# XiSHEN0220/RANSAC-Flow

Hardware: AMD Instinct MI355X
Metric: aligned image-pairs/sec @480×640, 1/2/4/8 MI355X; max-abs flow Δ vs ref (higher is better)
Workload: dtype f32

## Files before the change

ransac-flow_amd/csrc/stem.hip:

```cpp
#include "common.h"
#include "group.h"

namespace {

constexpr int TH = 4, TW = 16;
constexpr int CR = 2 * TH + 2, CC = 2 * TW + 2;
constexpr int PRW = CR + 2, PCL = CC + 2;
constexpr int CST = CC + 1;
constexpr int CPS = CR * CST + 1;
constexpr int NPX = CR * CC;
constexpr int NSUB = (NPX + 31) / 32;
constexpr int KKS = 14;
constexpr int MCH = 32;

struct StemArgs {
    const float* in; const float* wT; const float* scale; const float* shift; float* out;
    int N, H, W, Cout, Mpad, Ho, Wo, tilesH, tilesW, chGroups;
};

__device__ __forceinline__ int reflect1i(int i, int n) { return i < 0 ? -i : (i >= n ? 2 * n - 2 - i : i); }

__device__ __forceinline__ float umaxf(float x, float y) {
    const unsigned a = __float_as_uint(x), b = __float_as_uint(y);
    return __uint_as_float(a > b ? a : b);
}

__global__ __launch_bounds__(256) void stem_conv_maxblur_kernel(StemArgs a) {
    __shared__ float P[3][PRW][PCL];
    __shared__ float C[MCH * CPS];

    const int t = threadIdx.x, lane = t & 63, wave = t >> 6;
    const int lrow = lane >> 5, lcol = lane & 31;
    int bid = blockIdx.x;
    const int cg = bid % a.chGroups; bid /= a.chGroups;
    const int tw = bid % a.tilesW; bid /= a.tilesW;
    const int th = bid % a.tilesH;
    const int n = bid / a.tilesH;
    const int oh0 = th * TH, ow0 = tw * TW;
    const int cy0 = 2 * oh0 - 1, cx0 = 2 * ow0 - 1;
    const int m0 = cg * MCH;
    const size_t HW = (size_t)a.H * a.W;

    const float* inn = a.in + (size_t)n * 3 * HW;
    constexpr int NP = (3 * PRW * PCL + 255) / 256;
    float pv_[NP];
    bool pok[NP];
#pragma unroll
    for (int u = 0; u < NP; ++u) {
        const int idx = t + 256 * u;
        const int c = idx / (PRW * PCL), rem = idx - c * (PRW * PCL);
        const int pr = rem / PCL, pc = rem - pr * PCL;
        const int gy = cy0 - 1 + pr, gx = cx0 - 1 + pc;
        pok[u] = idx < 3 * PRW * PCL && (unsigned)gy < (unsigned)a.H && (unsigned)gx < (unsigned)a.W;
        pv_[u] = inn[pok[u] ? (size_t)c * HW + (size_t)gy * a.W + gx : 0];
    }
    float af[KKS];
#pragma unroll
    for (int kk = 0; kk < KKS; ++kk) af[kk] = a.wT[(size_t)(2 * kk + lrow) * a.Mpad + m0 + lcol];
    int koff[KKS];
#pragma unroll
    for (int kk = 0; kk < KKS; ++kk) {
        const int k = 2 * kk + lrow;
        const int c = k / 9, t9 = k - c * 9, kh = t9 / 3, kw = t9 - kh * 3;
        koff[kk] = k < 27 ? c * (PRW * PCL) + kh * PCL + kw : 0;
    }
    float sc[16], sh[16];
#pragma unroll
    for (int r = 0; r < 16; ++r) {
        const int ch = m0 + 4 * lrow + (r & 3) + 8 * (r >> 2);
        sc[r] = a.scale ? a.scale[ch] : 1.0f;
        sh[r] = a.shift ? a.shift[ch] : 0.0f;
    }
#pragma unroll
    for (int u = 0; u < NP; ++u)
        if (t + 256 * u < 3 * PRW * PCL) (&P[0][0][0])[t + 256 * u] = pok[u] ? pv_[u] : 0.0f;
    __syncthreads();

    const float* pf = &P[0][0][0];
    for (int s = wave; s < NSUB; s += 4) {
        const int p = s * 32 + lcol;
        const bool pv = p < NPX;
        const int pc = pv ? p : 0;
        const int py = pc / CC, px = pc - py * CC;
        const int pbase = py * PCL + px;
        f32x16 acc;
#pragma unroll
        for (int r = 0; r < 16; ++r) acc[r] = 0.0f;
#pragma unroll
        for (int kk = 0; kk < KKS; ++kk) {
            float b = pf[pbase + koff[kk]];
            if (kk == KKS - 1) b = lrow ? 0.0f : b;
            acc = __builtin_amdgcn_mfma_f32_32x32x2f32(af[kk], b, acc, 0, 0, 0);
        }
        if (pv) {
#pragma unroll
            for (int r = 0; r < 16; ++r) {
                float v = fmaf(acc[r], sc[r], sh[r]);
                v = v > 0.0f ? v : 0.0f;
                C[(4 * lrow + (r & 3) + 8 * (r >> 2)) * CPS + py * CST + px] = v;
            }
        }
    }
    __syncthreads();

    const float w3[3] = {0.25f, 0.5f, 0.25f};
    const int Hm = a.H - 1, Wm = a.W - 1;
    for (int b = t; b < MCH * (TH / 2) * (TW / 2); b += 256) {
        const int bx = b % (TW / 2), by = (b / (TW / 2)) % (TH / 2), ch = b / ((TW / 2) * (TH / 2));
        const int oh = oh0 + 2 * by, ow = ow0 + 2 * bx;
        if (oh >= a.Ho || ow >= a.Wo) continue;
        float* dst = a.out + ((size_t)n * a.Cout + m0 + ch) * a.Ho * a.Wo;
        const float* Cc = C + ch * CPS;
        const bool interior = oh >= 1 && 2 * oh + 3 <= Hm - 1 && ow >= 1 && 2 * ow + 3 <= Wm - 1 && oh + 1 < a.Ho && ow + 1 < a.Wo;
        if (interior) {
            const int ly = 2 * oh - 1 - cy0, lx = 2 * ow - 1 - cx0;
            float v[6][6];
#pragma unroll
            for (int y = 0; y < 6; ++y)
#pragma unroll
                for (int x = 0; x < 6; ++x) v[y][x] = Cc[(ly + y) * CST + lx + x];
            float hmx[5][6], M[5][5];
#pragma unroll
            for (int y = 0; y < 5; ++y)
#pragma unroll
                for (int x = 0; x < 6; ++x) hmx[y][x] = umaxf(v[y][x], v[y + 1][x]);
#pragma unroll
            for (int y = 0; y < 5; ++y)
#pragma unroll
                for (int x = 0; x < 5; ++x) M[y][x] = umaxf(hmx[y][x], hmx[y][x + 1]);
#pragma unroll
            for (int dy = 0; dy < 2; ++dy)
#pragma unroll
                for (int dx = 0; dx < 2; ++dx) {
                    float acc = 0.0f;
#pragma unroll
                    for (int i = 0; i < 3; ++i)
#pragma unroll
                        for (int j = 0; j < 3; ++j) acc = fmaf(M[2 * dy + i][2 * dx + j], w3[i] * w3[j], acc);
                    dst[(size_t)(oh + dy) * a.Wo + ow + dx] = acc;
                }
            continue;
        }
        for (int dy = 0; dy < 2; ++dy)
            for (int dx = 0; dx < 2; ++dx) {
                const int o_h = oh + dy, o_w = ow + dx;
                if (o_h >= a.Ho || o_w >= a.Wo) continue;
                float acc = 0.0f;
#pragma unroll
                for (int i = 0; i < 3; ++i) {
                    const int my = reflect1i(2 * o_h - 1 + i, Hm) - cy0;
#pragma unroll
                    for (int j = 0; j < 3; ++j) {
                        const int mx = reflect1i(2 * o_w - 1 + j, Wm) - cx0;
                        const float m = umaxf(umaxf(Cc[my * CST + mx], Cc[(my + 1) * CST + mx]), umaxf(Cc[my * CST + mx + 1], Cc[(my + 1) * CST + mx + 1]));
                        acc = fmaf(m, w3[i] * w3[j], acc);
                    }
                }
                dst[(size_t)o_h * a.Wo + o_w] = acc;
            }
    }
}


namespace r50 {
constexpr int TH = 5, TW = 16;
constexpr int CR = 2 * TH + 1, CC = 2 * TW + 1;
constexpr int PR = 2 * CR + 5, PCW = 2 * CC + 5;
constexpr int PHALF = 36, PST = 2 * PHALF + 2;
constexpr int CHALF = 17, CST = 40;
constexpr int NSUB = CR + 1;
constexpr int KKS = 74;
constexpr int MCH = 32;
__host__ __device__ constexpr int koff(int k) {
    return k >= 147 ? 0 : (k / 49) * (PR * PST) + ((k % 49) / 7) * PST + (((k % 49) % 7) & 1) * PHALF + (((k % 49) % 7) >> 1);
}
}

struct Stem7Args {
    const float* in; const float* wT; const float* scale; const float* shift; float* out;
    int N, H, W, Cout, Mpad, Hc, Wc, Hp, Wp, tilesH, tilesW, chGroups;
#ifdef RFX_TRACE
    long long* trace;
#endif
};
#ifdef RFX_TRACE
extern "C" long long* rfx_debug_trace_ptr();
#define RFX_STAMP7(i) do { if (threadIdx.x == 0 && a.trace) a.trace[(size_t)bx * 8 + (i)] = (long long)__builtin_amdgcn_s_memtime(); } while (0)
#else
#define RFX_STAMP7(i)
#endif

__device__ __forceinline__ void stem7_conv_maxpool_body(const Stem7Args& a, const unsigned bx) {
    constexpr int TH = r50::TH, TW = r50::TW, CR = r50::CR, CC = r50::CC, PR = r50::PR, PCW = r50::PCW, PHALF = r50::PHALF,
                  PST = r50::PST, CST = r50::CST, CHALF = r50::CHALF, NSUB = r50::NSUB, KKS = r50::KKS, MCH = r50::MCH;
    using r50::koff;
    __shared__ float P[3][PR][PST];
    __shared__ float C[MCH][CR][CST];

    const int t = threadIdx.x, lane = t & 63, wave = t >> 6;
    const int lrow = lane >> 5, lcol = lane & 31;
    int bid = (int)bx;
    const int cg_first = bid % a.chGroups;
    bid /= a.chGroups;
    const int tw = bid % a.tilesW; bid /= a.tilesW;
    const int th = bid % a.tilesH;
    const int n = bid / a.tilesH;
    const int oh0 = th * TH, ow0 = tw * TW;
    const int cy0 = 2 * oh0 - 1, cx0 = 2 * ow0 - 1;
    const int iy0 = 2 * cy0 - 3, ix0 = 2 * cx0 - 3;
    const size_t HW = (size_t)a.H * a.W;

    RFX_STAMP7(0);
    const float* inn = a.in + (size_t)n * 3 * HW;
    constexpr int NP = (3 * PR * PCW + 255) / 256;
    float pv_[NP];
    unsigned pok = 0;
    const int c_0 = t / (PR * PCW), rem_0 = t - c_0 * (PR * PCW), pr_0 = rem_0 / PCW, pc_0 = rem_0 - pr_0 * PCW;
    {
        int c = c_0, pr = pr_0, pc = pc_0;
#pragma unroll
        for (int u = 0; u < NP; ++u) {
            const int gy = iy0 + pr, gx = ix0 + pc;
            const bool ok = c < 3 && (unsigned)gy < (unsigned)a.H && (unsigned)gx < (unsigned)a.W;
            pok |= ok ? (1u << u) : 0u;
            pv_[u] = inn[ok ? (size_t)c * HW + (size_t)gy * a.W + gx : 0];
            pc += 256 % PCW; pr += 256 / PCW;
            if (pc >= PCW) { pc -= PCW; ++pr; }
            if (pr >= PR) { pr -= PR; ++c; }
        }
    }
    float af[KKS];
    __shared__ float s_bn[2][128];
    for (int c = t; c < a.Cout && c < 128; c += 256) {
        s_bn[0][c] = a.scale ? a.scale[c] : 1.0f;
        s_bn[1][c] = a.shift ? a.shift[c] : 0.0f;
    }
    auto load_weights = [&](int m0) {
        const float* wl = a.wT;
        asm volatile("" : "+s"(wl) :: "memory");
#pragma unroll
        for (int kk = 0; kk < KKS; ++kk) af[kk] = wl[(size_t)(2 * kk + lrow) * a.Mpad + m0 + lcol];
    };
    load_weights(cg_first * MCH);
    {
        int c = c_0, pr = pr_0, pc = pc_0;
#pragma unroll
        for (int u = 0; u < NP; ++u) {
            if (c < 3) P[c][pr][(pc & 1) * PHALF + (pc >> 1)] = ((pok >> u) & 1u) ? pv_[u] : 0.0f;
            pc += 256 % PCW; pr += 256 / PCW;
            if (pc >= PCW) { pc -= PCW; ++pr; }
            if (pr >= PR) { pr -= PR; ++c; }
        }
    }
    RFX_STAMP7(1);
    __syncthreads();
    RFX_STAMP7(2);

    auto channel_group = [&](const int cg) {
    const int m0 = cg * MCH;
    const float* pf = &P[0][0][0];
    for (int s = wave; s < NSUB; s += 4) {
        const bool pv = s < CR || lcol < CR;
        const int py = s < CR ? s : (lcol < CR ? lcol : 0), px = s < CR ? lcol : CC - 1;
        const int pbase = 2 * py * PST + px;
        f32x16 acc;
#pragma unroll
        for (int r = 0; r < 16; ++r) acc[r] = 0.0f;
#pragma unroll
        for (int kk = 0; kk < KKS; ++kk) {
            const int off = lrow ? koff(2 * kk + 1) : koff(2 * kk);
            float b = pf[pbase + off];
            if (kk == KKS - 1) b = lrow ? 0.0f : b;
            acc = __builtin_amdgcn_mfma_f32_32x32x2f32(af[kk], b, acc, 0, 0, 0);
        }
        if (pv) {
#pragma unroll
            for (int r = 0; r < 16; ++r) {
                const int chl = m0 + 4 * lrow + (r & 3) + 8 * (r >> 2);
                float v = fmaf(acc[r], s_bn[0][chl], s_bn[1][chl]);
                v = v > 0.0f ? v : 0.0f;
                C[4 * lrow + (r & 3) + 8 * (r >> 2)][py][(px & 1) * CHALF + (px >> 1)] = v;
            }
        }
    }
    RFX_STAMP7(3);
    __syncthreads();
    RFX_STAMP7(4);

    for (int o = t; o < MCH * TH * TW; o += 256) {
        const int owl = o % TW, ohl = (o / TW) % TH, ch = o / (TW * TH);
        const int oh = oh0 + ohl, ow = ow0 + owl;
        if (oh >= a.Hp || ow >= a.Wp) continue;
        float m = 0.0f;
#pragma unroll
        for (int i = 0; i < 3; ++i) {
            const int gy = cy0 + 2 * ohl + i;
#pragma unroll
            for (int j = 0; j < 3; ++j) {
                const int gx = cx0 + 2 * owl + j;
                const bool ok = (unsigned)gy < (unsigned)a.Hc && (unsigned)gx < (unsigned)a.Wc;
                const float v = C[ch][2 * ohl + i][(j & 1) * CHALF + owl + (j >> 1)];
                m = ok ? umaxf(m, v) : m;
            }
        }
        a.out[(((size_t)n * a.Cout + m0 + ch) * a.Hp + oh) * a.Wp + ow] = m;
    }
    RFX_STAMP7(5);
    };
#pragma unroll 1
    for (int cg = cg_first; cg < cg_first + 1; ++cg) channel_group(cg);
}

__global__ __launch_bounds__(256, 2) void stem7_conv_maxpool_kernel(Stem7Args a) {
    stem7_conv_maxpool_body(a, blockIdx.x);
}

__global__ __launch_bounds__(256, 2) void stem7_conv_maxpool_group_kernel(RfxGroupArgs<Stem7Args> g) {
    const unsigned y = blockIdx.y;
    if (blockIdx.x >= g.gx[y]) return;
    stem7_conv_maxpool_body(g.p[y], blockIdx.x);
}

static int stem7_group_launch(const void* blob, const unsigned* gx, int n, hipStream_t st) {
    return rfx_group_launch_impl<Stem7Args>(stem7_conv_maxpool_group_kernel, 256, blob, gx, n, st);
}

}

extern "C" int rfx_stem_conv3x3_maxblur_f32(const float* in, const float* wT, const float* scale, const float* shift,
                                            float* out, int N, int H, int W, int Cout, void* stream) {
    if (!in || !wT || !out || N <= 0 || H < 3 || W < 3 || Cout <= 0) return RFX_E_ARG;
    if (Cout % MCH != 0) return RFX_E_ARG;
    StemArgs a;
    a.in = in; a.wT = wT; a.scale = scale; a.shift = shift; a.out = out;
    a.N = N; a.H = H; a.W = W; a.Cout = Cout; a.Mpad = (Cout + 127) / 128 * 128;
    a.Ho = (H - 2) / 2 + 1; a.Wo = (W - 2) / 2 + 1;
    a.tilesH = (a.Ho + TH - 1) / TH; a.tilesW = (a.Wo + TW - 1) / TW; a.chGroups = Cout / MCH;
    const long long nwg = (long long)N * a.tilesH * a.tilesW * a.chGroups;
    if (nwg > 0x7fffffffLL) return RFX_E_LIMIT;
    hipLaunchKernelGGL(stem_conv_maxblur_kernel, dim3((unsigned)nwg), dim3(256), 0, rfx_stream(stream), a);
    RFX_LAUNCH_CHECK();
    return RFX_OK;
}

extern "C" int rfx_stem_conv7x7_maxpool_f32(const float* in, const float* wT, const float* scale, const float* shift,
                                            float* out, int N, int H, int W, int Cout, void* stream) {
    if (!in || !wT || !out || N <= 0 || H < 1 || W < 1 || Cout <= 0) return RFX_E_ARG;
    if (Cout % r50::MCH != 0) return RFX_E_ARG;
    if (Cout > 128) return RFX_E_LIMIT;
    Stem7Args a;
    a.in = in; a.wT = wT; a.scale = scale; a.shift = shift; a.out = out;
    a.N = N; a.H = H; a.W = W; a.Cout = Cout; a.Mpad = (Cout + 127) / 128 * 128;
    a.Hc = (H + 6 - 7) / 2 + 1; a.Wc = (W + 6 - 7) / 2 + 1;
    a.Hp = (a.Hc + 2 - 3) / 2 + 1; a.Wp = (a.Wc + 2 - 3) / 2 + 1;
    a.tilesH = (a.Hp + r50::TH - 1) / r50::TH; a.tilesW = (a.Wp + r50::TW - 1) / r50::TW; a.chGroups = Cout / r50::MCH;
    const long long nwg = (long long)N * a.tilesH * a.tilesW * a.chGroups;
    if (nwg > 0x7fffffffLL) return RFX_E_LIMIT;
#ifdef RFX_TRACE
    a.trace = rfx_debug_trace_ptr();
#endif
    if (rfx_group_recording()) return rfx_group_record(&stem7_group_launch, &a, sizeof(a), (unsigned)nwg);
    hipLaunchKernelGGL(stem7_conv_maxpool_kernel, dim3((unsigned)nwg), dim3(256), 0, rfx_stream(stream), a);
    RFX_LAUNCH_CHECK();
    return RFX_OK;
}
```

Baseline: 164.4.

## Loop channel groups inside stem blocks and fuse horizontal maxpool via DPP

Both stem kernels now stage each input tile into LDS once and loop over all channel groups inside one workgroup, instead of launching a separate workgroup per channel group that reloads the same patch. The next group's weights are prefetched during the pooling phase. The 7x7 stem also does the horizontal 3-wide max inside the MFMA epilogue using DPP row shifts, and keeps a small side buffer for tile-edge columns, which shrinks the LDS intermediate and the pooling pass. The cost is fewer workgroups (a factor of chGroups) and therefore less parallelism, plus an extra barrier per group.

```diff
diff --git a/ransac-flow_amd/csrc/stem.hip b/ransac-flow_amd/csrc/stem.hip
--- a/ransac-flow_amd/csrc/stem.hip
+++ b/ransac-flow_amd/csrc/stem.hip
@@ -32,13 +32,11 @@
     const int t = threadIdx.x, lane = t & 63, wave = t >> 6;
     const int lrow = lane >> 5, lcol = lane & 31;
     int bid = blockIdx.x;
-    const int cg = bid % a.chGroups; bid /= a.chGroups;
     const int tw = bid % a.tilesW; bid /= a.tilesW;
     const int th = bid % a.tilesH;
     const int n = bid / a.tilesH;
     const int oh0 = th * TH, ow0 = tw * TW;
     const int cy0 = 2 * oh0 - 1, cx0 = 2 * ow0 - 1;
-    const int m0 = cg * MCH;
     const size_t HW = (size_t)a.H * a.W;
 
     const float* inn = a.in + (size_t)n * 3 * HW;
@@ -55,8 +53,11 @@
         pv_[u] = inn[pok[u] ? (size_t)c * HW + (size_t)gy * a.W + gx : 0];
     }
     float af[KKS];
-#pragma unroll
-    for (int kk = 0; kk < KKS; ++kk) af[kk] = a.wT[(size_t)(2 * kk + lrow) * a.Mpad + m0 + lcol];
+    auto load_weights = [&](const int m0) {
+#pragma unroll
+        for (int kk = 0; kk < KKS; ++kk) af[kk] = a.wT[(size_t)(2 * kk + lrow) * a.Mpad + m0 + lcol];
+    };
+    load_weights(0);
     int koff[KKS];
 #pragma unroll
     for (int kk = 0; kk < KKS; ++kk) {
@@ -64,6 +65,17 @@
         const int c = k / 9, t9 = k - c * 9, kh = t9 / 3, kw = t9 - kh * 3;
         koff[kk] = k < 27 ? c * (PRW * PCL) + kh * PCL + kw : 0;
     }
+#pragma unroll
+    for (int u = 0; u < NP; ++u)
+        if (t + 256 * u < 3 * PRW * PCL) (&P[0][0][0])[t + 256 * u] = pok[u] ? pv_[u] : 0.0f;
+    __syncthreads();
+
+    const float* pf = &P[0][0][0];
+    const float w3[3] = {0.25f, 0.5f, 0.25f};
+    const int Hm = a.H - 1, Wm = a.W - 1;
+#pragma unroll 1
+    for (int cg = 0; cg < a.chGroups; ++cg) {
+    const int m0 = cg * MCH;
     float sc[16], sh[16];
 #pragma unroll
     for (int r = 0; r < 16; ++r) {
@@ -71,18 +83,13 @@
         sc[r] = a.scale ? a.scale[ch] : 1.0f;
         sh[r] = a.shift ? a.shift[ch] : 0.0f;
     }
-#pragma unroll
-    for (int u = 0; u < NP; ++u)
-        if (t + 256 * u < 3 * PRW * PCL) (&P[0][0][0])[t + 256 * u] = pok[u] ? pv_[u] : 0.0f;
-    __syncthreads();
-
-    const float* pf = &P[0][0][0];
     for (int s = wave; s < NSUB; s += 4) {
         const int p = s * 32 + lcol;
         const bool pv = p < NPX;
         const int pc = pv ? p : 0;
         const int py = pc / CC, px = pc - py * CC;
-        const int pbase = py * PCL + px;
+        int pbase = py * PCL + px;
+        asm volatile("" : "+v"(pbase));
         f32x16 acc;
 #pragma unroll
         for (int r = 0; r < 16; ++r) acc[r] = 0.0f;
@@ -102,9 +109,8 @@
         }
     }
     __syncthreads();
-
-    const float w3[3] = {0.25f, 0.5f, 0.25f};
-    const int Hm = a.H - 1, Wm = a.W - 1;
+    if (cg + 1 < a.chGroups) load_weights(m0 + MCH);
+
     for (int b = t; b < MCH * (TH / 2) * (TW / 2); b += 256) {
         const int bx = b % (TW / 2), by = (b / (TW / 2)) % (TH / 2), ch = b / ((TW / 2) * (TH / 2));
         const int oh = oh0 + 2 * by, ow = ow0 + 2 * bx;
@@ -159,6 +165,8 @@
                 dst[(size_t)o_h * a.Wo + o_w] = acc;
             }
     }
+    __syncthreads();
+    }
 }
 
 
@@ -167,7 +175,8 @@
 constexpr int CR = 2 * TH + 1, CC = 2 * TW + 1;
 constexpr int PR = 2 * CR + 5, PCW = 2 * CC + 5;
 constexpr int PHALF = 36, PST = 2 * PHALF + 2;
-constexpr int CHALF = 17, CST = 40;
+constexpr int HPS = CR * TW + 4;
+constexpr int SPS = 24;
 constexpr int NSUB = CR + 1;
 constexpr int KKS = 74;
 constexpr int MCH = 32;
@@ -185,23 +194,33 @@
 };
 #ifdef RFX_TRACE
 extern "C" long long* rfx_debug_trace_ptr();
-#define RFX_STAMP7(i) do { if (threadIdx.x == 0 && a.trace) a.trace[(size_t)bx * 8 + (i)] = (long long)__builtin_amdgcn_s_memtime(); } while (0)
+#define RFX_NOW7() ((long long)__builtin_amdgcn_s_memtime())
+#define RFX_STAMP7(i) do { if (threadIdx.x == 0 && a.trace) a.trace[(size_t)bx * 8 + (i)] = RFX_NOW7(); } while (0)
+#define RFX_PUT7(i, v) do { if (threadIdx.x == 0 && a.trace) a.trace[(size_t)bx * 8 + (i)] = (v); } while (0)
+#define RFX_TRACE7(x) x
 #else
 #define RFX_STAMP7(i)
+#define RFX_PUT7(i, v)
+#define RFX_TRACE7(x)
 #endif
 
+template <int N>
+__device__ __forceinline__ unsigned row_shl0(unsigned v) {
+    return (unsigned)__builtin_amdgcn_update_dpp(0, (int)v, 0x100 + N, 0xf, 0xf, true);
+}
+
 __device__ __forceinline__ void stem7_conv_maxpool_body(const Stem7Args& a, const unsigned bx) {
-    constexpr int TH = r50::TH, TW = r50::TW, CR = r50::CR, CC = r50::CC, PR = r50::PR, PCW = r50::PCW, PHALF = r50::PHALF,
-                  PST = r50::PST, CST = r50::CST, CHALF = r50::CHALF, NSUB = r50::NSUB, KKS = r50::KKS, MCH = r50::MCH;
+    constexpr int TH = r50::TH, TW = r50::TW, CR = r50::CR, PR = r50::PR, PCW = r50::PCW, PHALF = r50::PHALF,
+                  PST = r50::PST, HPS = r50::HPS, SPS = r50::SPS, NSUB = r50::NSUB, KKS = r50::KKS, MCH = r50::MCH;
     using r50::koff;
     __shared__ float P[3][PR][PST];
-    __shared__ float C[MCH][CR][CST];
+    __shared__ float Hx[MCH * HPS];
+    __shared__ float Sd[MCH * SPS];
+    __shared__ float s_bn[2][128];
 
     const int t = threadIdx.x, lane = t & 63, wave = t >> 6;
     const int lrow = lane >> 5, lcol = lane & 31;
     int bid = (int)bx;
-    const int cg_first = bid % a.chGroups;
-    bid /= a.chGroups;
     const int tw = bid % a.tilesW; bid /= a.tilesW;
     const int th = bid % a.tilesH;
     const int n = bid / a.tilesH;
@@ -229,19 +248,17 @@
             if (pr >= PR) { pr -= PR; ++c; }
         }
     }
-    float af[KKS];
-    __shared__ float s_bn[2][128];
     for (int c = t; c < a.Cout && c < 128; c += 256) {
         s_bn[0][c] = a.scale ? a.scale[c] : 1.0f;
         s_bn[1][c] = a.shift ? a.shift[c] : 0.0f;
     }
-    auto load_weights = [&](int m0) {
-        const float* wl = a.wT;
-        asm volatile("" : "+s"(wl) :: "memory");
-#pragma unroll
-        for (int kk = 0; kk < KKS; ++kk) af[kk] = wl[(size_t)(2 * kk + lrow) * a.Mpad + m0 + lcol];
+    float af[KKS];
+    auto load_weights = [&](const int m0) {
+        const unsigned voff = (unsigned)(lrow * a.Mpad + m0 + lcol);
+#pragma unroll
+        for (int kk = 0; kk < KKS; ++kk) af[kk] = (a.wT + (size_t)(2 * kk) * a.Mpad)[voff];
     };
-    load_weights(cg_first * MCH);
+    load_weights(0);
     {
         int c = c_0, pr = pr_0, pc = pc_0;
 #pragma unroll
@@ -255,14 +272,20 @@
     RFX_STAMP7(1);
     __syncthreads();
     RFX_STAMP7(2);
-
-    auto channel_group = [&](const int cg) {
+    RFX_TRACE7(long long tr_mark = RFX_NOW7(); long long tr_mfma = 0; long long tr_pool = 0;)
+
+    const float* pf = &P[0][0][0];
+#pragma unroll 1
+    for (int cg = 0; cg < a.chGroups; ++cg) {
     const int m0 = cg * MCH;
-    const float* pf = &P[0][0][0];
     for (int s = wave; s < NSUB; s += 4) {
-        const bool pv = s < CR || lcol < CR;
-        const int py = s < CR ? s : (lcol < CR ? lcol : 0), px = s < CR ? lcol : CC - 1;
-        const int pbase = 2 * py * PST + px;
+        const bool rowt = s < CR;
+        const int cl = lcol & 15;
+        const bool pv = rowt || cl < CR;
+        const int py = rowt ? s : (cl < CR ? cl : 0), px = rowt ? lcol : 16 + (lcol & 16);
+        int pbase = 2 * py * PST + px;
+        asm volatile("" : "+v"(pbase));
+        const bool ok = pv && (unsigned)(cy0 + py) < (unsigned)a.Hc && (unsigned)(cx0 + px) < (unsigned)a.Wc;
         f32x16 acc;
 #pragma unroll
         for (int r = 0; r < 16; ++r) acc[r] = 0.0f;
@@ -273,42 +296,56 @@
             if (kk == KKS - 1) b = lrow ? 0.0f : b;
             acc = __builtin_amdgcn_mfma_f32_32x32x2f32(af[kk], b, acc, 0, 0, 0);
         }
-        if (pv) {
+        if (rowt) {
+            unsigned hm[16];
 #pragma unroll
             for (int r = 0; r < 16; ++r) {
                 const int chl = m0 + 4 * lrow + (r & 3) + 8 * (r >> 2);
                 float v = fmaf(acc[r], s_bn[0][chl], s_bn[1][chl]);
                 v = v > 0.0f ? v : 0.0f;
-                C[4 * lrow + (r & 3) + 8 * (r >> 2)][py][(px & 1) * CHALF + (px >> 1)] = v;
+                const unsigned u = ok ? __float_as_uint(v) : 0u;
+                const unsigned u1 = row_shl0<1>(u), u2 = row_shl0<2>(u);
+                const unsigned m1 = u > u1 ? u : u1;
+                hm[r] = m1 > u2 ? m1 : u2;
             }
-        }
-    }
-    RFX_STAMP7(3);
-    __syncthreads();
-    RFX_STAMP7(4);
+            if (!(lcol & 1)) {
+#pragma unroll
+                for (int r = 0; r < 16; ++r)
+                    Hx[(4 * lrow + (r & 3) + 8 * (r >> 2)) * HPS + py * TW + (lcol >> 1)] = __uint_as_float(hm[r]);
+            }
+        } else if (pv) {
+#pragma unroll
+            for (int r = 0; r < 16; ++r) {
+                const int chl = m0 + 4 * lrow + (r & 3) + 8 * (r >> 2);
+                float v = fmaf(acc[r], s_bn[0][chl], s_bn[1][chl]);
+                v = v > 0.0f ? v : 0.0f;
+                Sd[(4 * lrow + (r & 3) + 8 * (r >> 2)) * SPS + (lcol >> 4) * 12 + py] = ok ? v : 0.0f;
+            }
+        }
+    }
+    __syncthreads();
+    RFX_TRACE7(const long long tr_a = RFX_NOW7(); tr_mfma += tr_a - tr_mark; tr_mark = tr_a;)
+    if (cg + 1 < a.chGroups) load_weights(m0 + MCH);
 
     for (int o = t; o < MCH * TH * TW; o += 256) {
         const int owl = o % TW, ohl = (o / TW) % TH, ch = o / (TW * TH);
         const int oh = oh0 + ohl, ow = ow0 + owl;
         if (oh >= a.Hp || ow >= a.Wp) continue;
-        float m = 0.0f;
-#pragma unroll
-        for (int i = 0; i < 3; ++i) {
-            const int gy = cy0 + 2 * ohl + i;
-#pragma unroll
-            for (int j = 0; j < 3; ++j) {
-                const int gx = cx0 + 2 * owl + j;
-                const bool ok = (unsigned)gy < (unsigned)a.Hc && (unsigned)gx < (unsigned)a.Wc;
-                const float v = C[ch][2 * ohl + i][(j & 1) * CHALF + owl + (j >> 1)];
-                m = ok ? umaxf(m, v) : m;
-            }
+        const float* hx = Hx + ch * HPS + 2 * ohl * TW + owl;
+        float m = umaxf(umaxf(hx[0], hx[TW]), hx[2 * TW]);
+        if ((owl & 7) == 7) {
+            const float* sd = Sd + ch * SPS + (owl >> 3) * 12 + 2 * ohl;
+            m = umaxf(m, umaxf(umaxf(sd[0], sd[1]), sd[2]));
         }
         a.out[(((size_t)n * a.Cout + m0 + ch) * a.Hp + oh) * a.Wp + ow] = m;
     }
+    __syncthreads();
+    RFX_TRACE7(const long long tr_b = RFX_NOW7(); tr_pool += tr_b - tr_mark; tr_mark = tr_b;)
+    }
+    RFX_PUT7(3, tr_mfma);
+    RFX_PUT7(4, tr_pool);
     RFX_STAMP7(5);
-    };
-#pragma unroll 1
-    for (int cg = cg_first; cg < cg_first + 1; ++cg) channel_group(cg);
+    RFX_PUT7(6, (long long)a.chGroups);
 }
 
 __global__ __launch_bounds__(256, 2) void stem7_conv_maxpool_kernel(Stem7Args a) {
@@ -336,7 +373,7 @@
     a.N = N; a.H = H; a.W = W; a.Cout = Cout; a.Mpad = (Cout + 127) / 128 * 128;
     a.Ho = (H - 2) / 2 + 1; a.Wo = (W - 2) / 2 + 1;
     a.tilesH = (a.Ho + TH - 1) / TH; a.tilesW = (a.Wo + TW - 1) / TW; a.chGroups = Cout / MCH;
-    const long long nwg = (long long)N * a.tilesH * a.tilesW * a.chGroups;
+    const long long nwg = (long long)N * a.tilesH * a.tilesW;
     if (nwg > 0x7fffffffLL) return RFX_E_LIMIT;
     hipLaunchKernelGGL(stem_conv_maxblur_kernel, dim3((unsigned)nwg), dim3(256), 0, rfx_stream(stream), a);
     RFX_LAUNCH_CHECK();
@@ -354,7 +391,7 @@
     a.Hc = (H + 6 - 7) / 2 + 1; a.Wc = (W + 6 - 7) / 2 + 1;
     a.Hp = (a.Hc + 2 - 3) / 2 + 1; a.Wp = (a.Wc + 2 - 3) / 2 + 1;
     a.tilesH = (a.Hp + r50::TH - 1) / r50::TH; a.tilesW = (a.Wp + r50::TW - 1) / r50::TW; a.chGroups = Cout / r50::MCH;
-    const long long nwg = (long long)N * a.tilesH * a.tilesW * a.chGroups;
+    const long long nwg = (long long)N * a.tilesH * a.tilesW;
     if (nwg > 0x7fffffffLL) return RFX_E_LIMIT;
 #ifdef RFX_TRACE
     a.trace = rfx_debug_trace_ptr();
```

New measurement: 166.3, median of 6. 1.01x the previous value.
